# FocoosAI/focoos

Measured on NVIDIA H100. Metric: images/sec fai-detr-l bs=32 640x640 inference, higher is better.
Workload: dtype f32 (storage and accumulation; every conv/linear product = 3 f16 wgmma products, error ~2^-21)

## Files before the change

### focoos_b200/csrc/conv_tc.cu

```cuda
#include <cuda.h>

#include <cstdlib>
#include <type_traits>

#include "common.cuh"
#include "wgmma.cuh"

namespace fb200 {

namespace tc {

constexpr int BLOCK_M = 128;
constexpr int STAGING_BYTES = BLOCK_M * 128;
constexpr int NUM_THREADS = 384;
constexpr int CONSUMER_WARPS = 8;

struct PairOut { __half hi, lo; };
template <typename T> struct is_pair { static constexpr bool value = false; };
template <> struct is_pair<PairOut> { static constexpr bool value = true; };

struct KParams {
  const float* scale; const float* bias; const void* res;
  int act, Cout;
  int KH, KW, pad, cchunks;
  int seg_chunks, lo_off;
  int w_seg;
  int BW, BH, tiles_w, tiles_h;
  int Ho, Wo;
  int x_pitch;
  int stride2;
  int num_k_blocks;
  int n_tiles, total_tiles;
  float* rowmax;
  int w_batched;
};

__device__ __forceinline__ uint32_t smem_u32(const void* p) { return (uint32_t)__cvta_generic_to_shared(p); }

__device__ __forceinline__ void mbar_init(uint64_t* bar, uint32_t count) {
  asm volatile("mbarrier.init.shared::cta.b64 [%0], %1;" ::"r"(smem_u32(bar)), "r"(count));
}
__device__ __forceinline__ void mbar_arrive_expect_tx(uint64_t* bar, uint32_t bytes) {
  asm volatile("mbarrier.arrive.expect_tx.shared::cta.b64 _, [%0], %1;" ::"r"(smem_u32(bar)), "r"(bytes) : "memory");
}
__device__ __forceinline__ void mbar_arrive(uint64_t* bar) {
  asm volatile("mbarrier.arrive.shared::cta.b64 _, [%0];" ::"r"(smem_u32(bar)) : "memory");
}
__device__ __forceinline__ void mbar_wait(uint64_t* bar, uint32_t parity) {
  uint32_t done = 0;
  uint32_t spins = 0;
  while (true) {
    asm volatile(
        "{\n\t.reg .pred p;\n\t"
        "mbarrier.try_wait.parity.shared::cta.b64 p, [%1], %2;\n\t"
        "selp.b32 %0, 1, 0, p;\n\t}"
        : "=r"(done)
        : "r"(smem_u32(bar)), "r"(parity)
        : "memory");
    if (done) break;
    if (++spins > (1u << 26)) __trap();
  }
}
__device__ __forceinline__ void fence_barrier_init() { asm volatile("fence.mbarrier_init.release.cluster;" ::: "memory"); }
__device__ __forceinline__ void fence_proxy_async() { asm volatile("fence.proxy.async.shared::cta;" ::: "memory"); }
__device__ __forceinline__ void consumer_bar() { asm volatile("bar.sync 1, 256;" ::: "memory"); }

__device__ __forceinline__ void tma_load_2d(const CUtensorMap* map, uint64_t* bar, void* dst, int c0, int c1) {
  asm volatile("cp.async.bulk.tensor.2d.shared::cluster.global.mbarrier::complete_tx::bytes [%0], [%1, {%3, %4}], [%2];"
               ::"r"(smem_u32(dst)), "l"(map), "r"(smem_u32(bar)), "r"(c0), "r"(c1) : "memory");
}
__device__ __forceinline__ void tma_load_3d(const CUtensorMap* map, uint64_t* bar, void* dst, int c0, int c1, int c2) {
  asm volatile("cp.async.bulk.tensor.3d.shared::cluster.global.mbarrier::complete_tx::bytes [%0], [%1, {%3, %4, %5}], [%2];"
               ::"r"(smem_u32(dst)), "l"(map), "r"(smem_u32(bar)), "r"(c0), "r"(c1), "r"(c2) : "memory");
}
__device__ __forceinline__ void tma_load_4d(const CUtensorMap* map, uint64_t* bar, void* dst, int c0, int c1, int c2, int c3) {
  asm volatile("cp.async.bulk.tensor.4d.shared::cluster.global.mbarrier::complete_tx::bytes [%0], [%1, {%3, %4, %5, %6}], [%2];"
               ::"r"(smem_u32(dst)), "l"(map), "r"(smem_u32(bar)), "r"(c0), "r"(c1), "r"(c2), "r"(c3) : "memory");
}
__device__ __forceinline__ void tma_load_5d(const CUtensorMap* map, uint64_t* bar, void* dst, int c0, int c1, int c2, int c3, int c4) {
  asm volatile("cp.async.bulk.tensor.5d.shared::cluster.global.mbarrier::complete_tx::bytes [%0], [%1, {%3, %4, %5, %6, %7}], [%2];"
               ::"r"(smem_u32(dst)), "l"(map), "r"(smem_u32(bar)), "r"(c0), "r"(c1), "r"(c2), "r"(c3), "r"(c4) : "memory");
}
__device__ __forceinline__ void tma_prefetch_4d(const CUtensorMap* map, int c0, int c1, int c2, int c3) {
  asm volatile("cp.async.bulk.prefetch.tensor.4d.L2.global [%0, {%1, %2, %3, %4}];" ::"l"(map), "r"(c0), "r"(c1), "r"(c2), "r"(c3) : "memory");
}
__device__ __forceinline__ void tma_prefetch_5d(const CUtensorMap* map, int c0, int c1, int c2, int c3, int c4) {
  asm volatile("cp.async.bulk.prefetch.tensor.5d.L2.global [%0, {%1, %2, %3, %4, %5}];" ::"l"(map), "r"(c0), "r"(c1), "r"(c2), "r"(c3), "r"(c4) : "memory");
}
__device__ __forceinline__ void tma_store_4d(const CUtensorMap* map, const void* src, int c0, int c1, int c2, int c3) {
  asm volatile("cp.async.bulk.tensor.4d.global.shared::cta.bulk_group [%0, {%2, %3, %4, %5}], [%1];"
               ::"l"(map), "r"(smem_u32(src)), "r"(c0), "r"(c1), "r"(c2), "r"(c3) : "memory");
}
__device__ __forceinline__ void tma_store_commit() { asm volatile("cp.async.bulk.commit_group;" ::: "memory"); }
template <int N> __device__ __forceinline__ void tma_store_wait_read() { asm volatile("cp.async.bulk.wait_group.read %0;" ::"n"(N) : "memory"); }
__device__ __forceinline__ void tma_store_wait_all() { asm volatile("cp.async.bulk.wait_group 0;" ::: "memory"); }

template <int BLOCK_K>
__device__ __forceinline__ uint64_t make_smem_desc(uint32_t smem_addr) {
  uint64_t d = 0;
  d |= (uint64_t)((smem_addr & 0x3FFFFu) >> 4);
  d |= (uint64_t)1 << 16;
  d |= (uint64_t)((8 * BLOCK_K * 2) >> 4) << 32;
  d |= (uint64_t)(BLOCK_K == 64 ? 1 : 2) << 62;
  return d;
}

template <bool GELU>
__device__ __forceinline__ float act1(float v, int act) {
  if constexpr (GELU) return 0.5f * v * (1.f + erff(v * 0.70710678118654752440f));
  switch (act & 15) {
    case FB200_ACT_RELU: return fmaxf(v, 0.f);
    case FB200_ACT_SILU: return __fdividef(v, 1.f + __expf(-v));
    default: return v;
  }
}

__device__ __forceinline__ void atomic_max_float(float* addr, float v) {
  if (v >= 0.f) atomicMax(reinterpret_cast<int*>(addr), __float_as_int(v));
  else atomicMin(reinterpret_cast<unsigned int*>(addr), __float_as_uint(v));
}

template <int BLOCK_K, bool FS> __host__ __device__ constexpr int a_stage_bytes() { return (FS ? 2 : 1) * BLOCK_M * BLOCK_K * 2; }
template <int BLOCK_N, int BLOCK_K, bool FS> __host__ __device__ constexpr int b_stage_bytes() { return (FS ? 2 : 1) * BLOCK_N * BLOCK_K * 2; }
template <int BLOCK_N, int STAGES, int BLOCK_K, int NSTG, bool FS> constexpr int smem_bytes() {
  return STAGES * (a_stage_bytes<BLOCK_K, FS>() + b_stage_bytes<BLOCK_N, BLOCK_K, FS>()) + NSTG * STAGING_BYTES + (2 * STAGES + 1) * 8 + 1024 ;
}

template <int BLOCK_N, int STAGES, typename TOut, int BLOCK_K, int NSTG, bool GELU, bool FS>
__global__ void __launch_bounds__(NUM_THREADS, 1)
conv_tc_kernel(const __grid_constant__ CUtensorMap tmap_a, const __grid_constant__ CUtensorMap tmap_b,
               const __grid_constant__ CUtensorMap tmap_d, const __grid_constant__ CUtensorMap tmap_r,
               const __grid_constant__ CUtensorMap tmap_d2, const __grid_constant__ CUtensorMap tmap_r2, const KParams p) {
  constexpr bool PAIR = is_pair<TOut>::value;
  static_assert(BLOCK_K == 32 || BLOCK_K == 64, "one swizzle row per channel chunk");
  extern __shared__ __align__(1024) uint8_t smem_raw[];
  uint8_t* smem = reinterpret_cast<uint8_t*>((reinterpret_cast<uintptr_t>(smem_raw) + 1023) & ~uintptr_t(1023));
  constexpr int A_STAGE_BYTES = a_stage_bytes<BLOCK_K, FS>();
  constexpr int B_STAGE_BYTES = b_stage_bytes<BLOCK_N, BLOCK_K, FS>();
  constexpr int A_HALF = BLOCK_M * BLOCK_K * 2;
  constexpr int B_HALF = BLOCK_N * BLOCK_K * 2;
  uint8_t* smem_a = smem;
  uint8_t* smem_b = smem + STAGES * A_STAGE_BYTES;
  uint8_t* staging = smem_b + STAGES * B_STAGE_BYTES;
  uint64_t* full_bar = reinterpret_cast<uint64_t*>(staging + NSTG * STAGING_BYTES);
  uint64_t* empty_bar = full_bar + STAGES;
  uint64_t* res_bar = empty_bar + STAGES;

  const int warp = threadIdx.x >> 5, lane = threadIdx.x & 31;
  if (threadIdx.x == 0) {
    asm volatile("prefetch.tensormap [%0];" ::"l"(&tmap_a) : "memory");
    asm volatile("prefetch.tensormap [%0];" ::"l"(&tmap_b) : "memory");
    asm volatile("prefetch.tensormap [%0];" ::"l"(&tmap_d) : "memory");
    for (int i = 0; i < STAGES; ++i) { mbar_init(&full_bar[i], 1); mbar_init(&empty_bar[i], CONSUMER_WARPS); }
    mbar_init(res_bar, 1);
    fence_barrier_init();
  }
  __syncthreads();
  const int tiles_per_img = p.tiles_w * p.tiles_h;
  struct TileXY { int n0, img, h0, w0; };
  auto tile_of = [&](int t) {
    TileXY r;
    r.n0 = (t % p.n_tiles) * BLOCK_N;
    const int mt = t / p.n_tiles;
    r.img = mt / tiles_per_img;
    const int rem = mt - r.img * tiles_per_img;
    r.h0 = (rem / p.tiles_w) * p.BH;
    r.w0 = (rem % p.tiles_w) * p.BW;
    return r;
  };

  if (warp < 4) {
    if (threadIdx.x != 0) return;
    const uint32_t a_bytes = (uint32_t)(p.BW * p.BH * BLOCK_K * 2);
    auto a_chan = [&](int cc) -> int {
      if (p.seg_chunks == 0) return cc * BLOCK_K;
      const int seg = cc / p.seg_chunks, within = cc - seg * p.seg_chunks;
      return (seg == 2 ? p.lo_off : 0) + within * BLOCK_K;
    };
    auto load_a = [&](uint64_t* bar, void* dst, int c, int kh, int kw, int h0, int w0, int img) {
      if (!p.stride2) {
        tma_load_4d(&tmap_a, bar, dst, c, w0 + kw - p.pad, h0 + kh - p.pad, img);
      } else {
        const int th = kh - p.pad, tw = kw - p.pad;
        tma_load_5d(&tmap_a, bar, dst, (tw & 1) * p.x_pitch + c, w0 + (tw >> 1), th & 1, h0 + (th >> 1), img);
      }
    };
    auto load_b = [&](uint64_t* bar, void* dst, int k, int n0, int img) {
      if (p.w_batched) tma_load_3d(&tmap_b, bar, dst, k, n0, img);
      else tma_load_2d(&tmap_b, bar, dst, k, n0);
    };
    int stage = 0;
    uint32_t phase = 0;
    for (int t = blockIdx.x; t < p.total_tiles; t += gridDim.x) {
      const TileXY tc = tile_of(t);
      {
        const int tn = t + gridDim.x;
        if (tn < p.total_tiles && (tn / p.n_tiles) != (t / p.n_tiles)) {
          const TileXY tnx = tile_of(tn);
          const int nchunks = FS ? 2 * p.cchunks : p.cchunks;
          for (int cc = 0; cc < nchunks; ++cc) {
            const int a_c0 = FS ? (cc < p.cchunks ? cc * BLOCK_K : p.lo_off + (cc - p.cchunks) * BLOCK_K) : a_chan(cc);
            if (!p.stride2) tma_prefetch_4d(&tmap_a, a_c0, tnx.w0, tnx.h0, tnx.img);
            else {
              for (int par = 0; par < 4; ++par)
                tma_prefetch_5d(&tmap_a, (par & 1) * p.x_pitch + a_c0, tnx.w0, par >> 1, tnx.h0, tnx.img);
            }
          }
        }
      }
      for (int kb = 0; kb < p.num_k_blocks; ++kb) {
        mbar_wait(&empty_bar[stage], phase ^ 1);
        const int tap = kb / p.cchunks, cc = kb - tap * p.cchunks;
        const int kh = tap / p.KW, kw = tap - kh * p.KW;
        uint8_t* dst_a = smem_a + stage * A_STAGE_BYTES;
        uint8_t* dst_b = smem_b + stage * B_STAGE_BYTES;
        if constexpr (FS) {
          const int k_hi = tap * 3 * p.w_seg + cc * BLOCK_K, k_lo = k_hi + p.w_seg;
          mbar_arrive_expect_tx(&full_bar[stage], 2u * a_bytes + (uint32_t)B_STAGE_BYTES);
          load_a(&full_bar[stage], dst_a, cc * BLOCK_K, kh, kw, tc.h0, tc.w0, tc.img);
          load_a(&full_bar[stage], dst_a + A_HALF, p.lo_off + cc * BLOCK_K, kh, kw, tc.h0, tc.w0, tc.img);
          load_b(&full_bar[stage], dst_b, k_hi, tc.n0, tc.img);
          load_b(&full_bar[stage], dst_b + B_HALF, k_lo, tc.n0, tc.img);
        } else {
          mbar_arrive_expect_tx(&full_bar[stage], a_bytes + (uint32_t)B_STAGE_BYTES);
          load_a(&full_bar[stage], dst_a, a_chan(cc), kh, kw, tc.h0, tc.w0, tc.img);
          load_b(&full_bar[stage], dst_b, kb * BLOCK_K, tc.n0, tc.img);
        }
        if (++stage == STAGES) { stage = 0; phase ^= 1; }
      }
    }
    return;
  }

  const int ct = threadIdx.x - 128;
  const int g = ct >> 7;
  const int r0 = g * 64 + ((ct & 127) >> 5) * 16 + (lane >> 2);
  const int cq = 2 * (lane & 3);
  constexpr int NACC = BLOCK_N / 2;
  constexpr int CHUNK_COLS = 128 / (int)sizeof(TOut);
  const bool post = (p.act & FB200_ACT_RESIDUAL_AFTER) != 0;
  const bool has_res = p.res != nullptr;
  float acc[NACC];
  int stage = 0;
  uint32_t phase = 0, res_phase = 0, chunk_ctr = 0;
  for (int t = blockIdx.x; t < p.total_tiles; t += gridDim.x) {
    const TileXY tc = tile_of(t);
    int prev = -1;
    for (int kb = 0; kb < p.num_k_blocks; ++kb) {
      mbar_wait(&full_bar[stage], phase);
      const uint32_t sa = smem_u32(smem_a + stage * A_STAGE_BYTES) + (uint32_t)(g * 64 * BLOCK_K * 2);
      const uint32_t sb = smem_u32(smem_b + stage * B_STAGE_BYTES);
      const uint64_t da = make_smem_desc<BLOCK_K>(sa), db = make_smem_desc<BLOCK_K>(sb);
      wgmma_fence();
#pragma unroll
      for (int k = 0; k < BLOCK_K / 16; ++k) {
        const uint64_t ko = (uint64_t)(k * 2);
        Wgmma<BLOCK_N, 0>::mma(acc, da + ko, db + ko, (kb > 0 || k > 0) ? 1u : 0u);
        if constexpr (FS) {
          const uint64_t da_lo = make_smem_desc<BLOCK_K>(sa + A_HALF), db_lo = make_smem_desc<BLOCK_K>(sb + B_HALF);
          Wgmma<BLOCK_N, 0>::mma(acc, da + ko, db_lo + ko, 1u);
          Wgmma<BLOCK_N, 0>::mma(acc, da_lo + ko, db + ko, 1u);
        }
      }
      wgmma_commit();
      wgmma_wait<1>();
      if (prev >= 0 && lane == 0) mbar_arrive(&empty_bar[prev]);
      prev = stage;
      if (++stage == STAGES) { stage = 0; phase ^= 1; }
    }
    wgmma_wait<0>();
    if (prev >= 0 && lane == 0) mbar_arrive(&empty_bar[prev]);

    auto scale_of = [&](int n) { return (p.scale && n < p.Cout) ? __ldg(p.scale + n) : 1.f; };
    auto bias_of = [&](int n) { return (p.bias && n < p.Cout) ? __ldg(p.bias + n) : 0.f; };
    auto row_valid = [&](int row, int64_t& pix) {
      const int bh = row / p.BW, bw = row - bh * p.BW;
      const int ho = tc.h0 + bh, wo = tc.w0 + bw;
      pix = ((int64_t)tc.img * p.Ho + ho) * p.Wo + wo;
      return row < p.BW * p.BH && ho < p.Ho && wo < p.Wo;
    };
    if (p.rowmax) {
      float m[2] = {-INFINITY, -INFINITY};
#pragma unroll
      for (int j = 0; j < BLOCK_N / 8; ++j) {
#pragma unroll
        for (int e = 0; e < 2; ++e) {
          const int n = tc.n0 + 8 * j + cq + e;
          if (n < p.Cout) {
            const float s = scale_of(n), b = bias_of(n);
            m[0] = fmaxf(m[0], fmaf(acc[4 * j + e], s, b));
            m[1] = fmaxf(m[1], fmaf(acc[4 * j + 2 + e], s, b));
          }
        }
      }
#pragma unroll
      for (int h = 0; h < 2; ++h) {
        m[h] = fmaxf(m[h], __shfl_xor_sync(0xffffffffu, m[h], 1));
        m[h] = fmaxf(m[h], __shfl_xor_sync(0xffffffffu, m[h], 2));
        int64_t pix;
        if ((lane & 3) == 0 && row_valid(r0 + 8 * h, pix)) atomic_max_float(p.rowmax + pix, m[h]);
      }
      continue;
    }
#pragma unroll
    for (int ch = 0; ch < (BLOCK_N + CHUNK_COLS - 1) / CHUNK_COLS; ++ch) {
      const int c0 = ch * CHUNK_COLS;
      if (tc.n0 + c0 >= p.Cout) break;
      uint8_t* stg = staging + (chunk_ctr % NSTG) * STAGING_BYTES;
      if (ct == 0) {
        tma_store_wait_read<NSTG - 1>();
        if (has_res) {
          mbar_arrive_expect_tx(res_bar, (uint32_t)(p.BW * p.BH * 128));
          tma_load_4d(&tmap_r, res_bar, stg, tc.n0 + c0, tc.w0, tc.h0, tc.img);
          if constexpr (PAIR) tma_load_4d(&tmap_r2, res_bar, stg + STAGING_BYTES / 2, tc.n0 + c0, tc.w0, tc.h0, tc.img);
        }
      }
      consumer_bar();
      if (has_res) { mbar_wait(res_bar, res_phase); res_phase ^= 1; }
#pragma unroll
      for (int jj = 0; jj < CHUNK_COLS / 8; ++jj) {
        const int j = c0 / 8 + jj;
        if (j >= BLOCK_N / 8) break;
        const int lc = 8 * jj + cq;
        const int n = tc.n0 + c0 + lc;
        const float s0 = scale_of(n), s1 = scale_of(n + 1), b0 = bias_of(n), b1 = bias_of(n + 1);
#pragma unroll
        for (int h = 0; h < 2; ++h) {
          const int row = r0 + 8 * h;
          float v0 = fmaf(acc[4 * j + 2 * h], s0, b0), v1 = fmaf(acc[4 * j + 2 * h + 1], s1, b1);
          int off;
          if constexpr (PAIR) off = row * 64 + ((((lc >> 3) ^ ((row >> 1) & 3)) << 4) | ((lc & 7) * 2));
          else if constexpr (sizeof(TOut) == 2) off = row * 128 + ((((lc >> 3) ^ (row & 7)) << 4) | ((lc & 7) * 2));
          else off = row * 128 + ((((lc >> 2) ^ (row & 7)) << 4) | ((lc & 3) * 4));
          auto add_residual = [&]() {
            if (!has_res) return;
            if constexpr (PAIR) {
              const float2 fh = __half22float2(*reinterpret_cast<const __half2*>(stg + off));
              const float2 fl = __half22float2(*reinterpret_cast<const __half2*>(stg + STAGING_BYTES / 2 + off));
              v0 += fh.x + fl.x;
              v1 += fh.y + fl.y;
            } else if constexpr (sizeof(TOut) == 2) {
              const float2 f = __half22float2(*reinterpret_cast<const __half2*>(stg + off));
              v0 += f.x;
              v1 += f.y;
            } else {
              const float2 f = *reinterpret_cast<const float2*>(stg + off);
              v0 += f.x;
              v1 += f.y;
            }
          };
          if (!post) add_residual();
          v0 = act1<GELU>(v0, p.act);
          v1 = act1<GELU>(v1, p.act);
          if (post) add_residual();
          if constexpr (PAIR) {
            const __half2 hi = __floats2half2_rn(v0, v1);
            const float2 hf = __half22float2(hi);
            *reinterpret_cast<__half2*>(stg + off) = hi;
            *reinterpret_cast<__half2*>(stg + STAGING_BYTES / 2 + off) = __floats2half2_rn(v0 - hf.x, v1 - hf.y);
          } else if constexpr (sizeof(TOut) == 2) {
            *reinterpret_cast<__half2*>(stg + off) = __floats2half2_rn(v0, v1);
          } else {
            *reinterpret_cast<float2*>(stg + off) = make_float2(v0, v1);
          }
        }
      }
      fence_proxy_async();
      consumer_bar();
      if (ct == 0) {
        tma_store_4d(&tmap_d, stg, tc.n0 + c0, tc.w0, tc.h0, tc.img);
        if constexpr (PAIR) tma_store_4d(&tmap_d2, stg + STAGING_BYTES / 2, tc.n0 + c0, tc.w0, tc.h0, tc.img);
        tma_store_commit();
      }
      ++chunk_ctr;
    }
  }
  if (ct == 0) tma_store_wait_all();
}

typedef CUresult (*EncodeTiledFn)(CUtensorMap*, CUtensorMapDataType, cuuint32_t, void*, const cuuint64_t*, const cuuint64_t*,
                                  const cuuint32_t*, const cuuint32_t*, CUtensorMapInterleave, CUtensorMapSwizzle,
                                  CUtensorMapL2promotion, CUtensorMapFloatOOBfill);
static EncodeTiledFn get_encode() {
  static EncodeTiledFn fn = nullptr;
  if (!fn) {
    void* p = nullptr;
    cudaDriverEntryPointQueryResult q;
    if (cudaGetDriverEntryPoint("cuTensorMapEncodeTiled", &p, cudaEnableDefault, &q) == cudaSuccess && q == cudaDriverEntryPointSuccess)
      fn = reinterpret_cast<EncodeTiledFn>(p);
  }
  return fn;
}

static int encode(CUtensorMap* m, CUtensorMapDataType dt, int elt, int rank, void* base, const uint64_t* dims, const uint64_t* strides_elts,
                  const uint32_t* box, const char* what, CUtensorMapSwizzle swz = CU_TENSOR_MAP_SWIZZLE_128B) {
  EncodeTiledFn fn = get_encode();
  if (!fn) { set_error("conv_tc: cuTensorMapEncodeTiled unavailable"); return FB200_ERR_CUDA; }
  cuuint64_t gdim[5], gstr[4];
  cuuint32_t bdim[5], estr[5];
  for (int i = 0; i < rank; ++i) { gdim[i] = dims[i]; bdim[i] = box[i]; estr[i] = 1; }
  for (int i = 1; i < rank; ++i) gstr[i - 1] = strides_elts[i] * (uint64_t)elt;
  CUresult r = fn(m, dt, (cuuint32_t)rank, base, gdim, gstr, bdim, estr, CU_TENSOR_MAP_INTERLEAVE_NONE, swz,
                  CU_TENSOR_MAP_L2_PROMOTION_L2_256B, CU_TENSOR_MAP_FLOAT_OOB_FILL_NONE);
  if (r != CUDA_SUCCESS) {
    set_error("conv_tc: cuTensorMapEncodeTiled(%s) failed with %d (rank %d dims %llu,%llu,%llu,%llu box %u,%u,%u,%u)", what, (int)r, rank,
              (unsigned long long)dims[0], (unsigned long long)dims[1], (unsigned long long)(rank > 2 ? dims[2] : 0),
              (unsigned long long)(rank > 3 ? dims[3] : 0), box[0], box[1], rank > 2 ? box[2] : 0, rank > 3 ? box[3] : 0);
    return FB200_ERR_CUDA;
  }
  return FB200_OK;
}

static void choose_tile(int Ho, int Wo, int* BW, int* BH) {
  double best = -1.0;
  for (int bw = 1; bw <= (Wo < 128 ? Wo : 128); ++bw) {
    int bh = 128 / bw;
    if (bh > Ho) bh = Ho;
    if (bh < 1) continue;
    const double tiles = (double)((Wo + bw - 1) / bw) * (double)((Ho + bh - 1) / bh);
    const double eff = (double)Wo * Ho / (tiles * 128.0);
    if (eff > best + 1e-9 || (eff > best - 1e-9 && bw > *BW)) { best = eff; *BW = bw; *BH = bh; }
  }
}

static int num_sms() {
  static int n = 0;
  if (!n) {
    int dev = 0;
    cudaGetDevice(&dev);
    cudaDeviceGetAttribute(&n, cudaDevAttrMultiProcessorCount, dev);
    if (n <= 0) n = 132;
  }
  return n;
}

template <int BLOCK_N, int STAGES, typename TOut, int BLOCK_K, int NSTG, bool GELU, bool FS = false>
static int launch(const CUtensorMap& ta, const CUtensorMap& tb, const CUtensorMap& td, const CUtensorMap& tr, const CUtensorMap& td2, const CUtensorMap& tr2,
                  const KParams& kp, cudaStream_t st) {
  auto kern = conv_tc_kernel<BLOCK_N, STAGES, TOut, BLOCK_K, NSTG, GELU, FS>;
  constexpr int smem = smem_bytes<BLOCK_N, STAGES, BLOCK_K, NSTG, FS>();
  static_assert(smem <= 227 * 1024, "shared memory budget exceeded");
  static bool configured = false;
  if (!configured) {
    cudaError_t e = cudaFuncSetAttribute(kern, cudaFuncAttributeMaxDynamicSharedMemorySize, smem);
    if (e != cudaSuccess) { set_error("conv_tc: cudaFuncSetAttribute(%d B) failed: %s", smem, cudaGetErrorString(e)); return FB200_ERR_CUDA; }
    configured = true;
  }
  const int64_t cap = num_sms();
  const unsigned grid = (unsigned)(kp.total_tiles < cap ? kp.total_tiles : cap);
  kern<<<grid, NUM_THREADS, smem, st>>>(ta, tb, td, tr, td2, tr2, kp);
  FB_CHECK_LAUNCH("conv_tc_kernel");
  return FB200_OK;
}

}

bool conv2d_tc_supported(const ConvParams& p, int x_dtype, int out_dtype) {
  if (x_dtype != FB200_F16) return false;
  if (out_dtype != FB200_F16 && out_dtype != FB200_F32 && out_dtype != FB200_F16PAIR) return false;
  const int Clog = p.split3 ? p.Cin / 3 : p.Cin;
  if (out_dtype == FB200_F16PAIR) {
    if (!p.split3 || p.rowmax || p.w_bs != 0 || p.Cout % 8 != 0) return false;
    if ((p.out_lo_off * 2) % 16 != 0 || (p.out_pitch * 2) % 16 != 0 || (p.out_bs * 2) % 16 != 0) return false;
    if (p.res && ((p.res_lo_off * 2) % 16 != 0 || (p.res_pitch * 2) % 16 != 0 || p.Cout % 32 != 0)) return false;
  }
  if (p.split3 && p.x_lo_off && (p.x_lo_off * 2) % 16 != 0) return false;
  if (Clog % 32 != 0 || p.x_pitch % 8 != 0) return false;
  if (p.split3 && p.Cin % 3 != 0) return false;
  if ((reinterpret_cast<uintptr_t>(p.x) | reinterpret_cast<uintptr_t>(p.w) | reinterpret_cast<uintptr_t>(p.out)) & 15) return false;
  const int oelt = out_dtype == FB200_F32 ? 4 : 2;
  if ((p.out_pitch * oelt) % 16 != 0) return false;
  if (p.res && ((p.res_pitch * oelt) % 16 != 0 || (reinterpret_cast<uintptr_t>(p.res) & 15))) return false;
  if (p.res && out_dtype != FB200_F16PAIR && p.Cout % (128 / oelt) != 0) return false;
  if (p.KH != p.KW) return false;
  if (p.w_bs != 0 && (p.w_bs * 2) % 16 != 0) return false;
  if ((p.act & 15) == FB200_ACT_GELU && (out_dtype != FB200_F16 || Clog % 64 != 0)) return false;
  if ((p.act & 15) == FB200_ACT_SIGMOID) return false;
  if ((p.out_bs * oelt) % 16 != 0) return false;
  if (p.stride == 1) return (2 * p.pad == p.KH - 1) || (p.KH == 1 && p.pad == 0);
  if (p.stride == 2) return ((p.KH == 3 && p.pad == 1) || (p.KH == 2 && p.pad == 0)) && p.H % 2 == 0 && p.W % 2 == 0;
  return false;
}

int conv2d_tc(const ConvParams& p, cudaStream_t st) {
  using namespace tc;
  KParams kp;
  kp.scale = p.scale; kp.bias = p.bias; kp.res = p.res; kp.act = p.act; kp.Cout = p.Cout;
  kp.KH = p.KH; kp.KW = p.KW; kp.pad = p.pad;
  const int Clog = p.split3 ? p.Cin / 3 : p.Cin;
  const int BK = (Clog % 64 == 0) ? 64 : 32;
  kp.seg_chunks = p.split3 ? Clog / BK : 0;
  kp.lo_off = (p.split3 && p.x_lo_off) ? (int)p.x_lo_off : Clog;
  kp.w_seg = Clog;
  const CUtensorMapSwizzle swz = BK == 64 ? CU_TENSOR_MAP_SWIZZLE_128B : CU_TENSOR_MAP_SWIZZLE_64B;
  kp.cchunks = p.Cin / BK; kp.x_pitch = p.x_pitch;
  kp.stride2 = (p.stride == 2) ? 1 : 0;
  kp.num_k_blocks = p.KH * p.KW * kp.cchunks;
  int B = p.B, H = p.H, W = p.W, Ho = p.Ho, Wo = p.Wo;
  const bool flat = (p.KH == 1 && p.stride == 1 && p.out_bs == (int64_t)p.Ho * p.Wo * p.out_pitch) && p.w_bs == 0;
  kp.w_batched = p.w_bs != 0 ? 1 : 0;
  kp.rowmax = p.rowmax;
  if (flat) {
    if (p.M > 0x7fffffffLL) { set_error("conv_tc: M too large"); return FB200_ERR_UNSUPPORTED; }
    W = Wo = (int)p.M; H = Ho = 1; B = 1;
  }
  int BW = 1, BH = 1;
  choose_tile(Ho, Wo, &BW, &BH);
  kp.BW = BW; kp.BH = BH; kp.tiles_w = (Wo + BW - 1) / BW; kp.tiles_h = (Ho + BH - 1) / BH; kp.Ho = Ho; kp.Wo = Wo;
  const int64_t m_tiles = (int64_t)B * kp.tiles_w * kp.tiles_h;

  CUtensorMap ta, tb, td;
  int rc;
  const uint64_t P = (uint64_t)p.x_pitch;
  if (!kp.stride2) {
    const uint64_t dims[4] = {(uint64_t)(p.split3 ? kp.lo_off + Clog : p.Cin), (uint64_t)W, (uint64_t)H, (uint64_t)B};
    const uint64_t str[4] = {1, P, P * W, P * W * H};
    const uint32_t box[4] = {(uint32_t)BK, (uint32_t)BW, (uint32_t)BH, 1};
    rc = encode(&ta, CU_TENSOR_MAP_DATA_TYPE_FLOAT16, 2, 4, const_cast<void*>(p.x), dims, str, box, "A", swz);
  } else {
    const uint64_t dims[5] = {2 * P, (uint64_t)W / 2, 2, (uint64_t)H / 2, (uint64_t)B};
    const uint64_t str[5] = {1, 2 * P, P * W, 2 * P * W, P * W * H};
    const uint32_t box[5] = {(uint32_t)BK, (uint32_t)BW, 1, (uint32_t)BH, 1};
    rc = encode(&ta, CU_TENSOR_MAP_DATA_TYPE_FLOAT16, 2, 5, const_cast<void*>(p.x), dims, str, box, "A(s2)", swz);
  }
  if (rc) return rc;

  auto run = [&](auto blockn_tag, auto stages_tag, auto bk_tag, auto gelu_tag, auto fs_tag) -> int {
    constexpr bool FS_ = decltype(fs_tag)::value;
    constexpr int BN_ = decltype(blockn_tag)::value;
    constexpr int ST_ = decltype(stages_tag)::value;
    constexpr int BK_ = decltype(bk_tag)::value;
    constexpr int NS_ = 2;
    {
      const uint64_t dims[3] = {(uint64_t)p.K, (uint64_t)p.Cout, (uint64_t)p.B};
      const uint64_t str[3] = {1, (uint64_t)p.K, (uint64_t)p.w_bs};
      const uint32_t box[3] = {(uint32_t)BK_, (uint32_t)BN_, 1};
      int r2 = encode(&tb, CU_TENSOR_MAP_DATA_TYPE_FLOAT16, 2, p.w_bs ? 3 : 2, const_cast<void*>(p.w), dims, str, box, "W", swz);
      if (r2) return r2;
    }
    const bool out16 = p.out_dtype == FB200_F16;
    const bool outp = p.out_dtype == FB200_F16PAIR;
    CUtensorMap tr, td2, tr2;
    if (outp) {
      const uint64_t OP = (uint64_t)p.out_pitch;
      const uint64_t dims[4] = {(uint64_t)p.Cout, (uint64_t)Wo, (uint64_t)Ho, (uint64_t)B};
      const uint64_t str[4] = {1, OP, OP * Wo, flat ? OP * Wo * Ho : (uint64_t)p.out_bs};
      const uint32_t box[4] = {32, (uint32_t)BW, (uint32_t)BH, 1};
      int r2 = encode(&td, CU_TENSOR_MAP_DATA_TYPE_FLOAT16, 2, 4, p.out, dims, str, box, "D(hi)", CU_TENSOR_MAP_SWIZZLE_64B);
      if (r2) return r2;
      r2 = encode(&td2, CU_TENSOR_MAP_DATA_TYPE_FLOAT16, 2, 4, static_cast<__half*>(p.out) + p.out_lo_off, dims, str, box, "D(lo)", CU_TENSOR_MAP_SWIZZLE_64B);
      if (r2) return r2;
      tr = td; tr2 = td2;
      if (p.res) {
        const uint64_t RP = (uint64_t)p.res_pitch;
        const uint64_t rstr[4] = {1, RP, RP * Wo, RP * Wo * Ho};
        r2 = encode(&tr, CU_TENSOR_MAP_DATA_TYPE_FLOAT16, 2, 4, const_cast<void*>(p.res), dims, rstr, box, "R(hi)", CU_TENSOR_MAP_SWIZZLE_64B);
        if (r2) return r2;
        r2 = encode(&tr2, CU_TENSOR_MAP_DATA_TYPE_FLOAT16, 2, 4, const_cast<__half*>(static_cast<const __half*>(p.res)) + p.res_lo_off, dims, rstr, box, "R(lo)", CU_TENSOR_MAP_SWIZZLE_64B);
        if (r2) return r2;
      }
    } else {
      const uint64_t OP = (uint64_t)p.out_pitch;
      const uint64_t dims[4] = {(uint64_t)p.Cout, (uint64_t)Wo, (uint64_t)Ho, (uint64_t)B};
      const uint64_t str[4] = {1, OP, OP * Wo, flat ? OP * Wo * Ho : (uint64_t)p.out_bs};
      const uint32_t box[4] = {(uint32_t)(out16 ? 64 : 32), (uint32_t)BW, (uint32_t)BH, 1};
      int r2 = encode(&td, out16 ? CU_TENSOR_MAP_DATA_TYPE_FLOAT16 : CU_TENSOR_MAP_DATA_TYPE_FLOAT32, out16 ? 2 : 4, 4, p.out, dims, str, box, "D");
      if (r2) return r2;
      td2 = td; tr = td; tr2 = td;
      if (p.res) {
        const uint64_t RP = (uint64_t)p.res_pitch;
        const uint64_t rstr[4] = {1, RP, RP * Wo, RP * Wo * Ho};
        r2 = encode(&tr, out16 ? CU_TENSOR_MAP_DATA_TYPE_FLOAT16 : CU_TENSOR_MAP_DATA_TYPE_FLOAT32, out16 ? 2 : 4, 4, const_cast<void*>(p.res), dims, rstr, box, "R");
        if (r2) return r2;
      }
    }
    KParams k2 = kp;
    if constexpr (FS_) {
      k2.cchunks = Clog / BK_;
      k2.num_k_blocks = p.KH * p.KW * k2.cchunks;
      k2.seg_chunks = 0;
    }
    k2.n_tiles = (p.Cout + BN_ - 1) / BN_;
    const int64_t total = m_tiles * k2.n_tiles;
    if (total > 0x7fffffffLL) { set_error("conv_tc: too many tiles (%lld)", (long long)total); return FB200_ERR_UNSUPPORTED; }
    k2.total_tiles = (int)total;
    if constexpr (decltype(gelu_tag)::value) return launch<BN_, ST_, __half, BK_, NS_, true>(ta, tb, td, tr, td2, tr2, k2, st);
    else if constexpr (FS_) {
      if (outp) return launch<BN_, ST_, PairOut, BK_, NS_, false, true>(ta, tb, td, tr, td2, tr2, k2, st);
      return launch<BN_, ST_, float, BK_, NS_, false, true>(ta, tb, td, tr, td2, tr2, k2, st);
    } else {
      if (outp) { set_error("conv_tc: pair output is only produced by the fused-split configurations"); return FB200_ERR_UNSUPPORTED; }
      if (out16) return launch<BN_, ST_, __half, BK_, NS_, false>(ta, tb, td, tr, td2, tr2, k2, st);
      return launch<BN_, ST_, float, BK_, NS_, false>(ta, tb, td, tr, td2, tr2, k2, st);
    }
  };
  using std::integral_constant;
  typedef std::false_type NF;
  typedef std::true_type FS;
  typedef integral_constant<int, 64> K64;
  typedef integral_constant<int, 32> K32;
  typedef integral_constant<int, 128> N128;
  typedef integral_constant<int, 64> N64;
  typedef integral_constant<int, 4> S4;
  typedef integral_constant<int, 3> S3;
  if ((p.act & 15) == FB200_ACT_GELU)
    return run(N128{}, S4{}, K64{}, std::true_type{}, NF{});
  if (p.split3 && (p.out_dtype == FB200_F32 || p.out_dtype == FB200_F16PAIR)) {
    if (BK == 64) {
      if (p.Cout > 64) return run(N128{}, S3{}, K64{}, std::false_type{}, FS{});
      return run(N64{}, S4{}, K64{}, std::false_type{}, FS{});
    }
    if (p.Cout > 64) return run(N128{}, S4{}, K32{}, std::false_type{}, FS{});
    return run(N64{}, S4{}, K32{}, std::false_type{}, FS{});
  }
  if (BK == 32) {
    if (p.Cout > 64) return run(N128{}, S4{}, K32{}, std::false_type{}, NF{});
    return run(N64{}, S4{}, K32{}, std::false_type{}, NF{});
  }
  if (p.Cout > 64) return run(N128{}, S4{}, K64{}, std::false_type{}, NF{});
  return run(N64{}, S4{}, K64{}, std::false_type{}, NF{});
}

}
```

Before: 619.5.

## Prefetch residual tiles through the operand pipeline ring via the producer warp

```diff
diff --git a/focoos_b200/csrc/conv_tc.cu b/focoos_b200/csrc/conv_tc.cu
--- a/focoos_b200/csrc/conv_tc.cu
+++ b/focoos_b200/csrc/conv_tc.cu
@@ -146,13 +146,24 @@
   uint64_t* empty_bar = full_bar + STAGES;
   uint64_t* res_bar = empty_bar + STAGES;
 
+  constexpr int CHUNK_COLS = 128 / (int)sizeof(TOut);
+  constexpr int NCHUNKS = (BLOCK_N + CHUNK_COLS - 1) / CHUNK_COLS;
+  constexpr int RES_SLOTS_A = A_STAGE_BYTES / STAGING_BYTES;
+  constexpr int RES_SLOTS = RES_SLOTS_A + B_STAGE_BYTES / STAGING_BYTES;
+  constexpr bool RES_RING = RES_SLOTS > 0;
+  const bool res_ring = RES_RING && p.res != nullptr && p.rowmax == nullptr;
+  auto res_slot = [&](int s, int slot) -> uint8_t* {
+    return slot < RES_SLOTS_A ? smem_a + s * A_STAGE_BYTES + slot * STAGING_BYTES : smem_b + s * B_STAGE_BYTES + (slot - RES_SLOTS_A) * STAGING_BYTES;
+  };
+  auto chunks_of = [&](int n0) { return min(NCHUNKS, (p.Cout - n0 + CHUNK_COLS - 1) / CHUNK_COLS); };
+
   const int warp = threadIdx.x >> 5, lane = threadIdx.x & 31;
   if (threadIdx.x == 0) {
     asm volatile("prefetch.tensormap [%0];" ::"l"(&tmap_a) : "memory");
     asm volatile("prefetch.tensormap [%0];" ::"l"(&tmap_b) : "memory");
     asm volatile("prefetch.tensormap [%0];" ::"l"(&tmap_d) : "memory");
     for (int i = 0; i < STAGES; ++i) { mbar_init(&full_bar[i], 1); mbar_init(&empty_bar[i], CONSUMER_WARPS); }
-    mbar_init(res_bar, 1);
+    if constexpr (!RES_RING) mbar_init(res_bar, 1);
     fence_barrier_init();
   }
   __syncthreads();
@@ -228,6 +239,22 @@
         }
         if (++stage == STAGES) { stage = 0; phase ^= 1; }
       }
+      if constexpr (RES_RING) if (res_ring) {
+        const int nch = chunks_of(tc.n0);
+        for (int ch = 0; ch < nch; ++ch) {
+          const int slot = ch % RES_SLOTS;
+          if (slot == 0) {
+            mbar_wait(&empty_bar[stage], phase ^ 1);
+            mbar_arrive_expect_tx(&full_bar[stage], (uint32_t)(min(RES_SLOTS, nch - ch) * p.BW * p.BH * 128));
+          }
+          uint8_t* dst = res_slot(stage, slot);
+          tma_load_4d(&tmap_r, &full_bar[stage], dst, tc.n0 + ch * CHUNK_COLS, tc.w0, tc.h0, tc.img);
+          if constexpr (PAIR) tma_load_4d(&tmap_r2, &full_bar[stage], dst + STAGING_BYTES / 2, tc.n0 + ch * CHUNK_COLS, tc.w0, tc.h0, tc.img);
+          if (slot == RES_SLOTS - 1 || ch == nch - 1) {
+            if (++stage == STAGES) { stage = 0; phase ^= 1; }
+          }
+        }
+      }
     }
     return;
   }
@@ -237,7 +264,6 @@
   const int r0 = g * 64 + ((ct & 127) >> 5) * 16 + (lane >> 2);
   const int cq = 2 * (lane & 3);
   constexpr int NACC = BLOCK_N / 2;
-  constexpr int CHUNK_COLS = 128 / (int)sizeof(TOut);
   const bool post = (p.act & FB200_ACT_RESIDUAL_AFTER) != 0;
   const bool has_res = p.res != nullptr;
   float acc[NACC];
@@ -302,21 +328,31 @@
       }
       continue;
     }
+    const int nch = chunks_of(tc.n0);
 #pragma unroll
-    for (int ch = 0; ch < (BLOCK_N + CHUNK_COLS - 1) / CHUNK_COLS; ++ch) {
+    for (int ch = 0; ch < NCHUNKS; ++ch) {
       const int c0 = ch * CHUNK_COLS;
-      if (tc.n0 + c0 >= p.Cout) break;
+      if (ch >= nch) break;
       uint8_t* stg = staging + (chunk_ctr % NSTG) * STAGING_BYTES;
+      const uint8_t* res = stg;
       if (ct == 0) {
         tma_store_wait_read<NSTG - 1>();
-        if (has_res) {
+        if constexpr (!RES_RING) if (has_res) {
           mbar_arrive_expect_tx(res_bar, (uint32_t)(p.BW * p.BH * 128));
           tma_load_4d(&tmap_r, res_bar, stg, tc.n0 + c0, tc.w0, tc.h0, tc.img);
           if constexpr (PAIR) tma_load_4d(&tmap_r2, res_bar, stg + STAGING_BYTES / 2, tc.n0 + c0, tc.w0, tc.h0, tc.img);
         }
       }
       consumer_bar();
-      if (has_res) { mbar_wait(res_bar, res_phase); res_phase ^= 1; }
+      if constexpr (RES_RING) {
+        if (res_ring) {
+          if (ch % RES_SLOTS == 0) mbar_wait(&full_bar[stage], phase);
+          res = res_slot(stage, ch % RES_SLOTS);
+        }
+      } else if (has_res) {
+        mbar_wait(res_bar, res_phase);
+        res_phase ^= 1;
+      }
 #pragma unroll
       for (int jj = 0; jj < CHUNK_COLS / 8; ++jj) {
         const int j = c0 / 8 + jj;
@@ -335,16 +371,16 @@
           auto add_residual = [&]() {
             if (!has_res) return;
             if constexpr (PAIR) {
-              const float2 fh = __half22float2(*reinterpret_cast<const __half2*>(stg + off));
-              const float2 fl = __half22float2(*reinterpret_cast<const __half2*>(stg + STAGING_BYTES / 2 + off));
+              const float2 fh = __half22float2(*reinterpret_cast<const __half2*>(res + off));
+              const float2 fl = __half22float2(*reinterpret_cast<const __half2*>(res + STAGING_BYTES / 2 + off));
               v0 += fh.x + fl.x;
               v1 += fh.y + fl.y;
             } else if constexpr (sizeof(TOut) == 2) {
-              const float2 f = __half22float2(*reinterpret_cast<const __half2*>(stg + off));
+              const float2 f = __half22float2(*reinterpret_cast<const __half2*>(res + off));
               v0 += f.x;
               v1 += f.y;
             } else {
-              const float2 f = *reinterpret_cast<const float2*>(stg + off);
+              const float2 f = *reinterpret_cast<const float2*>(res + off);
               v0 += f.x;
               v1 += f.y;
             }
@@ -363,6 +399,13 @@
           } else {
             *reinterpret_cast<float2*>(stg + off) = make_float2(v0, v1);
           }
+        }
+      }
+      if constexpr (RES_RING) {
+        if (res_ring && (ch % RES_SLOTS == RES_SLOTS - 1 || ch == nch - 1)) {
+          __syncwarp();
+          if (lane == 0) mbar_arrive(&empty_bar[stage]);
+          if (++stage == STAGES) { stage = 0; phase ^= 1; }
         }
       }
       fence_proxy_async();
```

Result: faster. 640.2, median of 6 (+3.3%).
